# psaegert/bcnf

Hardware: AMD Instinct MI355X
Metric: NLL-training samples/sec + log_prob max-abs-err vs ref, trajectory_FC_small (higher is better)
Workload: dtype f32; 1 GPU; trajectory_FC_small NLL training step (configs[1]); batch_per_gpu=4096, global_batch=4096, parallelism=dp1, hip_graph=True, n_blocks=32, n_conditions=80

## Files before the change

bcnf_amd/csrc/bcnf_stack.hip:

```cpp
#include "bcnf_device.h"
#include "../../include/bcnf_amd.h"

#include <math.h>
#include <stdlib.h>
#include <string.h>

#include <algorithm>
#include <utility>
#include <vector>


#ifdef BCNF_PHASE_STAMPS
#define BCNF_STAMPS 1
#else
#define BCNF_STAMPS 0
#endif

namespace {

constexpr int NC16_MAX = 16;
constexpr int TILE = 256;
__host__ __device__ constexpr int tile_slot(int r, int q) { return 4 * r + ((q + (r >> 1)) & 3); }
__host__ __device__ constexpr int tile_ix(int s, int r) { return 4 * tile_slot(r, s & 3) + (s >> 2); }
__host__ __device__ constexpr int sample_of(int t8) { return (t8 >> 6) + 4 * ((t8 >> 4) & 3); }
// ... 855 lines not shown
#pragma unroll
    for (int e = 0; e < 8; ++e) {
      const int i4 = tid + 256 * e, r = i4 >> 5, col = (i4 & 31) * 4;
      if (col < L.Cp) *reinterpret_cast<floatx4*>(Bs + r * hs + col) = rv[e];
    }
#pragma unroll
    for (int kk = 0; kk < 2; ++kk) {
      const floatx4 v = va[kk] * am[kk];
#pragma unroll
      for (int q = 0; q < 4; ++q) As[(kk * 16 + j4 + q) * KHP + row] = v[q];
    }
    for (int c0 = KC; c0 < L.Cp; c0 += KC) {
      rows64_issue<VEC>(h, m1, L.C, L.ldh, m0 + KH * half, c0, rv);
      rows64_mask(m1, L.C, m0 + KH * half, c0, rv, ones);
#pragma unroll
      for (int e = 0; e < 8; ++e) {
        const int i4 = tid + 256 * e, r = i4 >> 5, col = c0 + (i4 & 31) * 4;
        if (col < L.Cp) *reinterpret_cast<floatx4*>(Bs + r * hs + col) = rv[e];
      }
    }
    __syncthreads();
#pragma unroll
    for (int j = 0; j < NT; ++j) {
      const int n = n_lo + j;
      if (n >= n_hi) continue;
#pragma unroll
      for (int t0 = 0; t0 < KH / 4; t0 += 8) {
        float a[8], bv[8];
#pragma unroll
        for (int t = 0; t < 8; ++t) {
          a[t] = As[(16 * kw + lr) * KHP + 4 * (t0 + t) + lq];
          bv[t] = Bs[(4 * (t0 + t) + lq) * hs + 16 * n + lr];
        }
#pragma unroll
        for (int t = 0; t < 8; t += 2) {
          acc[j] = mfma4(a[t], bv[t], acc[j]);
          acc1[j] = mfma4(a[t + 1], bv[t + 1], acc1[j]);
        }
      }
    }
  }
  if (k >= L.nb) return;
  float* o = work + (((long long)s * L.nb + k) * 16) * L.Cp;
#pragma unroll
  for (int j = 0; j < NT; ++j) {
    const int n = n_lo + j;
    if (n >= n_hi) continue;
    const floatx4 r = acc[j] + acc1[j];
#pragma unroll
    for (int i = 0; i < 4; ++i) o[(long long)(4 * lq + i) * L.Cp + 16 * n + lr] = r[i];
  }
}
size_t dw1h_half_lds_bytes(const BcnfLayout& L) {
  return sizeof(float) * (size_t)(32 * KHP + KH * bstride16(L.Cp));
}

__global__ __launch_bounds__(BCNF_WG) void k_dw1h_reduce(BcnfLayout L, const float* __restrict__ work, int splits,
                                                         float* __restrict__ dparams) {
  const long long per = 16LL * L.Cp, total = (long long)L.nb * per;
  const long long i = (long long)blockIdx.x * BCNF_WG + threadIdx.x;
  if (i >= total) return;
  const int k = (int)(i / per);
  const int rem = (int)(i - (long long)k * per);
  const int j = rem / L.Cp, c = rem - j * L.Cp;
  if (j >= L.H[1] || c >= L.C) return;
  float acc = 0.f;
  int s = 0;
  for (; s + 8 <= splits; s += 8) {
    float v[8];
#pragma unroll
    for (int t = 0; t < 8; ++t) v[t] = work[(long long)(s + t) * total + i];
#pragma unroll
    for (int t = 0; t < 8; ++t) acc += v[t];
  }
  for (; s < splits; ++s) acc += work[(long long)s * total + i];
  dparams[coupling_base(L, k) + L.lin_w[1] + j * L.lin_in[1] + L.Da + c] = acc;
}

__device__ __forceinline__ void gx_reduce_body(long long total, const float* __restrict__ work, int splits,
                                               float* __restrict__ gx, long long i) {
  if (i >= total) return;
  float acc = 0.f;
  int s = 0;
  for (; s + 16 <= splits; s += 16) {
    float v[16];
#pragma unroll
    for (int t = 0; t < 16; ++t) v[t] = work[(long long)(s + t) * total + i];
#pragma unroll
    for (int t = 0; t < 16; ++t) acc += v[t];
  }
  for (; s < splits; ++s) acc += work[(long long)s * total + i];
  gx[i] = acc;
}

__global__ __launch_bounds__(BCNF_WG) void k_fold_gx(long long total, const float* __restrict__ work, int splits,
                                                     float* __restrict__ gx) {
  gx_reduce_body(total, work, splits, gx, (long long)blockIdx.x * BCNF_WG + threadIdx.x);
}

struct RedShare {
  const float* slab;
  long long stride;
  int nwg;
  int own, first;
  float* dparams;
};
enum RedAdam { RED_NO_ADAM, RED_ADAM_DERIVED, RED_ADAM_PUBLISHED };
template <RedAdam AM>
__device__ __forceinline__ void reduce_share(const BcnfLayout& L, const RedShare& R, const FoldAdamArgs& A,
                                             float* __restrict__ smem);

__device__ __forceinline__ int c0_of_finish(int bx, int nct) { return (bx % nct) * 16; }

constexpr int FIN_KC = 512;
constexpr int FIN_SMEM = 2 * FIN_KC * 16;

__device__ __forceinline__ void tile16_accum(const float* __restrict__ As, const float* __restrict__ Bs, int kn,
                                             floatx4 (&acc)[4]) {
  const int lane = threadIdx.x & 63, ks = lane & 15, rb = lane >> 4, cb = threadIdx.x >> 6;
#pragma unroll 4
  for (int k = ks; k < kn; k += 16) {
    const floatx4 a = *reinterpret_cast<const floatx4*>(As + k * 16 + 4 * rb);
    const floatx4 b = *reinterpret_cast<const floatx4*>(Bs + k * 16 + 4 * cb);
#pragma unroll
    for (int r = 0; r < 4; ++r)
#pragma unroll
      for (int c = 0; c < 4; ++c) acc[r][c] = fmaf(a[r], b[c], acc[r][c]);
  }
}

__device__ __forceinline__ float tile16_reduce(float* __restrict__ red, const floatx4 (&acc)[4]) {
  const int lane = threadIdx.x & 63, ks = lane & 15, rb = lane >> 4, cb = threadIdx.x >> 6;
  __syncthreads();
#pragma unroll
  for (int r = 0; r < 4; ++r)
#pragma unroll
    for (int c = 0; c < 4; ++c) red[ks * 256 + (4 * rb + r) * 16 + 4 * cb + c] = acc[r][c];
  __syncthreads();
  float v = 0.f;
#pragma unroll
  for (int q = 0; q < 16; ++q) v += red[q * 256 + threadIdx.x];
  return v;
}

__global__ __launch_bounds__(BCNF_WG) void k_fold_finish(BcnfLayout L, const float* __restrict__ pk,
                                                         const float* __restrict__ gx, const float* __restrict__ wf,
                                                         const float* __restrict__ bf, int X,
                                                         float* __restrict__ dparams, float* __restrict__ dwf,
                                                         float* __restrict__ dbf, FoldAdamArgs A, RedShare R) {
  extern __shared__ __attribute__((aligned(16))) float smem[];
  if ((int)blockIdx.x >= R.own) {
    reduce_share<RED_ADAM_PUBLISHED>(L, R, A, smem);
    return;
  }
  float* As = smem;
  float* Bs = smem + FIN_KC * 16;
  const int Xp = fold_xp(X), tid = threadIdx.x, nct = L.Cp >> 4;
  floatx4 acc[4];
#pragma unroll
  for (int q = 0; q < 4; ++q) acc[q] = floatx4{0.f, 0.f, 0.f, 0.f};
  const bool adam = A.on && !(A.guard && A.guard[BCNF_GUARD_HALTED]);
  AdamScalars as{};
  const bool keeper = adam && blockIdx.x == 0 && tid == 0;
  const bool logger = keeper && A.log_values && A.log_history;
  long long log_row = 0;
  float step0 = 0.f, log_v[3];
  if (adam) {
    as = adam_scalars_of(A, A.asc[0], A.asc[1]);
    if (keeper) {
      log_row = A.cursor ? A.cursor[0] : 0LL;
      step0 = A.step[0];
    }
    if (logger) {
#pragma unroll
      for (int i = 0; i < 3; ++i) log_v[i] = A.log_values[i];
    }
  }
  int slot = -1;
  long long idx = 0;
  float ap = 0.f, am = 0.f, av = 0.f;
  if ((int)blockIdx.x < L.nb * nct) {
    const int j = tid >> 4, c = c0_of_finish(blockIdx.x, nct) + (tid & 15), k = blockIdx.x / nct;
    if (j < L.H[1] && c < L.C) {
      slot = 0;
      idx = coupling_base(L, k) + L.lin_w[1] + j * L.lin_in[1] + L.Da + c;
    }
  } else {
    const int tile = blockIdx.x - L.nb * nct, c = (tile % nct) * 16 + (tid >> 4), x = (tile / nct) * 16 + (tid & 15);
    if (c < L.C) {
      if (x < X) {
        slot = 1;
        idx = (long long)c * X + x;
      } else if (x == X && dbf) {
        slot = 2;
        idx = c;
      }
    }
  }
  float *sp = nullptr, *sm = nullptr, *sv = nullptr;
  if (adam) {
    if (slot == 0) {
      sp = A.p[0]; sm = A.m[0]; sv = A.v[0];
    } else if (slot == 1) {
      sp = A.p[1]; sm = A.m[1]; sv = A.v[1];
    } else if (slot == 2) {
      sp = A.p[2]; sm = A.m[2]; sv = A.v[2];
    }
  }
  if (sp) {
    ap = sp[idx];
    am = sm[idx];
    av = sv[idx];
  }
  auto finish_elem = [&](float gval) {
    if (!sp) return;
    adam_elem(ap, gval, am, av, as);
    sp[idx] = ap;
    sm[idx] = am;
    sv[idx] = av;
  };
  auto arrive = [&]() {
    if (!keeper) return;
    if (logger) __threadfence_system();
    A.step[0] = step0 + 1.0f;
    if (A.cursor) {
      const long long c = log_row + 1;
      A.cursor[0] = c < A.n_batches ? c : 0;
    }
  };
  if ((int)blockIdx.x < L.nb * nct) {
    const int k = blockIdx.x / nct, c0 = (blockIdx.x % nct) * 16;
    const float* g = gx + (long long)k * 16 * Xp;
    float va[16], vb[16];
#pragma unroll
    for (int e = 0; e < 16; ++e) {
      const int i = tid + BCNF_WG * e;
      const int j = i / Xp, xc = i - j * Xp, c = c0 + j;
      const bool in = i < 16 * Xp;
      va[e] = in ? g[i] : 0.f;
      float v = 0.f;
      if (in && c < L.C) v = xc < X ? wf[(long long)c * X + xc] : ((xc == X && bf) ? bf[c] : 0.f);
      vb[e] = v;
    }
#pragma unroll
    for (int e = 0; e < 16; ++e) {
      const int i = tid + BCNF_WG * e;
      if (i < 16 * Xp) {
        const int j = i / Xp, xc = i - j * Xp;
        As[xc * 16 + j] = va[e];
        Bs[xc * 16 + j] = vb[e];
      }
    }
    __syncthreads();
    if (logger) {
#pragma unroll
      for (int i = 0; i < 3; ++i)
        __hip_atomic_store(A.log_history + 3 * log_row + i, log_v[i], __ATOMIC_RELAXED, __HIP_MEMORY_SCOPE_SYSTEM);
    }
    tile16_accum(As, Bs, Xp, acc);
    const float v = tile16_reduce(smem, acc);
    const int j = tid >> 4, c = c0 + (tid & 15);
    if (j < L.H[1] && c < L.C) dparams[coupling_base(L, k) + L.lin_w[1] + j * L.lin_in[1] + L.Da + c] = v;
    finish_elem(v);
    __syncthreads();
    arrive();
    return;
  }
  const int tile = blockIdx.x - L.nb * nct, c0 = (tile % nct) * 16, x0 = (tile / nct) * 16;
  const int K = L.nb * 16;
  const float* w1r = pk + L.w1r_off + c0;
  for (int k0 = 0; k0 < K; k0 += FIN_KC) {
    const int kn = min(FIN_KC, K - k0);
    if (k0) __syncthreads();
    floatx4 va[FIN_KC * 4 / BCNF_WG], vb[FIN_KC * 4 / BCNF_WG];
#pragma unroll
    for (int e = 0; e < FIN_KC * 4 / BCNF_WG; ++e) {
      const int i4 = tid + BCNF_WG * e, r = i4 >> 2, q = i4 & 3, kj = k0 + (r < kn ? r : 0);
      va[e] = *reinterpret_cast<const floatx4*>(w1r + (long long)kj * L.Cp + 4 * q);
      vb[e] = *reinterpret_cast<const floatx4*>(gx + (long long)kj * Xp + x0 + 4 * q);
    }
#pragma unroll
    for (int e = 0; e < FIN_KC * 4 / BCNF_WG; ++e) {
      const int i4 = tid + BCNF_WG * e;
      reinterpret_cast<floatx4*>(As)[i4] = va[e];
      reinterpret_cast<floatx4*>(Bs)[i4] = vb[e];
    }
    __syncthreads();
    tile16_accum(As, Bs, kn, acc);
  }
  const float v = tile16_reduce(smem, acc);
  const int c = c0 + (tid >> 4), x = x0 + (tid & 15);
  if (c < L.C) {
    if (x < X) {
      if (dwf) dwf[(long long)c * X + x] = v;
    } else if (x == X && dbf) {
      dbf[c] = v;
    }
  }
  finish_elem(v);
  __syncthreads();
  arrive();
}

template <int NH>
struct RecF {
  static constexpr int B1 = 4, W1 = 8, HID = 24, T = 24 + 17 * (NH - 1), S = T + 17;
  static constexpr int Q = (S + 17 + 3) & ~3, MLP_END = (S + 17 + 3) & ~3, USED = Q + 64;
};
template <int NH>
struct RecB {
  static constexpr int AN = 0, QT = 4, TT = 68, ST = 84, HID = 100, W1T = 100 + 16 * (NH - 1);
  static constexpr int USED = W1T + 16;
};
template <int NH>
struct ActRec {
  static constexpr int YA = 2 * NH, YB = 2 * NH + 1, S = 2 * NH + 2;
  static constexpr int AR = 2 * NH + 3, AR4 = AR / 4, AR1 = AR - 4 * AR4;
  __host__ __device__ static constexpr int act(int l) { return 2 * l; }
  __host__ __device__ static constexpr int gd(int l) { return 2 * l + 1; }
  __host__ __device__ static constexpr int ready_layer(int q) {
    int r = 0;
    for (int i = 4 * q; i < 4 * q + 4; ++i) {
      const int li = i < 2 * NH ? i / 2 + 1 : (i == S ? NH + 1 : 0);
      r = li > r ? li : r;
    }
    return r;
  }
};

template <int LO, int HI>
__device__ __forceinline__ void ld_rec(float* __restrict__ rr, const float* __restrict__ R) {
  static_assert(LO % 4 == 0 && HI % 4 == 0, "record slices are 16-B aligned");
  const floatx4* R4 = reinterpret_cast<const floatx4*>(R + LO);
#pragma unroll
  for (int i = 0; i < (HI - LO) / 4; ++i) {
    const floatx4 v = R4[i];
    rr[LO + 4 * i + 0] = v.x;
// ... 1182 lines not shown
    for (int k = nb - 1; k >= 0; --k) {
      const int cur = k & 1;
      float gs[4 * BWD_G4];
      {
        const floatx4* gd4 = gsl + cur * BWD_G4 * BCNF_WG + tid;
#pragma unroll
        for (int i = 0; i < BWD_G4; ++i) {
          const floatx4 v = gd4[i * BCNF_WG];
          gs[4 * i] = v[0];
          gs[4 * i + 1] = v[1];
          gs[4 * i + 2] = v[2];
          gs[4 * i + 3] = v[3];
        }
      }
      float* Tt = dT + cur * J::ND * TILE + tix;
      const float* R = recB + cur * RING + j * L.RB;
      float rb[RBk::USED];
      ld_rec<0, RBk::HID>(rb, R);
      __builtin_amdgcn_sched_barrier(0);
      const float* gd = gs;
      const float S = gs[NH], ya = gs[NH + 1], yb = gs[NH + 2];
      const float an_sa = rb[RBk::AN], an_sb = rb[RBk::AN + 2], an_bb = rb[RBk::AN + 3];
      const float xb = fmaf(an_sb, yb, an_bb);
      const float e = exp_fast(S);
      float gza, gzb;
      if (QBC_DEV(L, QBC_MIX)) mix_bc(rb + RBk::QT, gya, gyb, gza, gzb);
      else mix(rb + RBk::QT, gya, gyb, gza, gzb);
      ld16(rb + RBk::HID, R + RBk::HID);
      __builtin_amdgcn_sched_barrier(0);
      const float dT_ = gzb;
      const float dS = (j < Db) ? fmaf(gzb * e, xb, dl) : 0.f;
      const float dSp = dS * (1.f - S * S);
      const float dxb = gzb * e;
      Tt[NH * TILE] = dT_;
      Tt[(NH + 1) * TILE] = dSp;
      float da = 0.f, da2 = 0.f;
      if (QBC_DEV(L, QBC_HEAD)) bc9x2(dT_, rb + RBk::TT, da, dSp, rb + RBk::ST, da2);
      else rot16x2(dT_, rb + RBk::TT, da, dSp, rb + RBk::ST, da2);
      da += da2;
#pragma unroll
      for (int l = NH; l >= 2; --l) {
        ld16(rb + RBk::HID + 16 * (NH - l + 1), R + RBk::HID + 16 * (NH - l + 1));
        __builtin_amdgcn_sched_barrier(0);
        const float dpre = da * gd[l - 1];
        Tt[(l - 1) * TILE] = dpre;
        da = rot16(dpre, rb + RBk::HID + 16 * (NH - l), 0.f);
      }
      const float dpre1 = da * gd[0];
      Tt[0] = dpre1;
      *(valid ? d1l + k * hps : d1_dummy) = dpre1;
      const float dxa = rot16(dpre1, rb + RBk::W1T, gza);
      {
        const float inv_a = (j < Da) ? __builtin_amdgcn_rcpf(an_sa) : 0.f;
        const float inv_b = (j < Db) ? __builtin_amdgcn_rcpf(an_sb) : 0.f;
        Tt[(NH + 2) * TILE] = fmaf(dxa, ya, dl * inv_a);
        Tt[(NH + 3) * TILE] = dxa;
        Tt[(NH + 4) * TILE] = fmaf(dxb, yb, dl * inv_b);
        Tt[(NH + 5) * TILE] = dxb;
      }
      gya = an_sa * dxa;
      gyb = an_sb * dxb;
      PHS(1)
      __syncthreads();
      PHS(2)
    }
    if (dy && valid) {
      if (j < Da) dy[b * D + j] = gya;
      if (j < Db) dy[b * D + Da + j] = gyb;
    }
  }
#if BCNF_STAMPS
  if (blockIdx.x == 0 && (threadIdx.x == 0 || threadIdx.x == BCNF_WG))
    for (int i = 0; i < 4; ++i) g_phase[(helper ? 4 : 0) + i] = ph_acc[i];
#endif
#undef PHS
  if (loss_out && blockIdx.x == 0) {
    __syncthreads();
    nll_finalize<BWD_WG>(nll_part, (int)gridDim.x, B, loss_out, rng_w, guard, dT);
  }
}

template <int N>
__device__ __forceinline__ int lpick(const int (&a)[N], int i) {
  int r = a[0];
#pragma unroll
  for (int t = 1; t < N; ++t) r = (i == t) ? a[t] : r;
  return r;
}

__device__ __forceinline__ long long slab_to_canonical(const BcnfLayout& L, int m, int o) {
  const int NH = L.NH, NW = NH + 2;
  const int cb = m * L.blk_stride + ((m < L.nb - 1) ? L.an_size : 0);
  if (o < NW * 256) {
    const int c = o >> 8, e = o & 255, lane = e >> 2;
    const int row = 4 * (lane >> 4) + (e & 3), col = lane & 15;
    const int l = c < NH ? c + 1 : NH + 1;
    const int nrows = c < NH ? lpick(L.H, l) : L.Db, ncols = (l == 1) ? L.Da : lpick(L.H, l - 1);
    if (row >= nrows || col >= ncols) return -1;
    const int row0 = (c == NH + 1) ? L.Db : 0;
    return (long long)cb + lpick(L.lin_w, l) + (row0 + row) * lpick(L.lin_in, l) + col;
  }
  const int o2 = o - NW * 256, c = o2 >> 4, r = o2 & 15;
  if (c < NH) return r < lpick(L.H, c + 1) ? (long long)cb + lpick(L.lin_b, c + 1) + r : -1;
  if (c < NH + 2) return r < L.Db ? (long long)cb + lpick(L.lin_b, NH + 1) + ((c == NH + 1) ? L.Db : 0) + r : -1;
  const int a = c - NH - 2;
  if (a >= 4 || !L.act_norm || m >= L.nb - 1 || r >= ((a < 2) ? L.Da : L.Db)) return -1;
  return (long long)m * L.blk_stride + ((a & 1) ? L.D : 0) + ((a < 2) ? 0 : L.Da) + r;
}

constexpr int RED_G = 8, RED_O4 = 32, RED_T = 16;

constexpr int RED_SMEM = RED_G * RED_O4 * 4 + 4;

template <RedAdam AM>
__device__ __forceinline__ void reduce_body(const BcnfLayout& L, const float* __restrict__ slab, long long stride,
                                            int nwg, float* __restrict__ out, int bx, float* __restrict__ smem,
                                            const FoldAdamArgs* A = nullptr) {
  floatx4 (*part)[RED_O4] = reinterpret_cast<floatx4 (*)[RED_O4]>(smem);
  float* sc = smem + RED_G * RED_O4 * 4;
  const int g = threadIdx.x / RED_O4, o4 = threadIdx.x % RED_O4;
  const long long i = ((long long)bx * RED_O4 + o4) * 4;
  const bool live = i < stride;
  const long long ic = live ? i : 0;
  const int m = (int)(ic / L.sblk), o = (int)(ic - (long long)m * L.sblk);
  long long ci[4];
  float ap[4], am[4], av[4];
  const float step0 = AM == RED_ADAM_DERIVED ? A->step[0] : 0.f;
  float pub[2] = {0.f, 0.f};
  if (AM == RED_ADAM_PUBLISHED && g == 0) {
    pub[0] = A->asc[0];
    pub[1] = A->asc[1];
  }
#pragma unroll
  for (int e = 0; e < 4; ++e) {
    ci[e] = slab_to_canonical(L, m, o + e);
    if (AM != RED_NO_ADAM && g == 0) {
      const long long c = ci[e] >= 0 ? ci[e] : 0;
      ap[e] = A->p[0][c];
      am[e] = A->m[0][c];
      av[e] = A->v[0][c];
    }
  }
  bool scalars_due = AM == RED_ADAM_DERIVED;
  auto scalars = [&]() {
    const double t = (double)(step0 + 1.0f);
    if (threadIdx.x == 0) sc[0] = (float)(A->lr / (1.0 - pow(A->b1, t)));
    if (threadIdx.x == 64) sc[1] = (float)sqrt(1.0 - pow(A->b2, t));
    scalars_due = false;
  };
  floatx4 acc = {0.f, 0.f, 0.f, 0.f};
  int w = g;
  for (; w + RED_G * (RED_T - 1) < nwg; w += RED_G * RED_T) {
    floatx4 v[RED_T];
#pragma unroll
    for (int t = 0; t < RED_T; ++t)
      v[t] = *reinterpret_cast<const floatx4*>(slab + (long long)(w + RED_G * t) * stride + ic);
    if (scalars_due) scalars();
#pragma unroll
    for (int t = 0; t < RED_T; ++t) acc += v[t];
  }
  for (; w < nwg; w += RED_G) acc += *reinterpret_cast<const floatx4*>(slab + (long long)w * stride + ic);
  if (scalars_due) scalars();
  part[g][o4] = acc;
  __syncthreads();
  if (g != 0 || !live) return;
  floatx4 tot = part[0][o4];
#pragma unroll
  for (int q = 1; q < RED_G; ++q) tot += part[q][o4];
  AdamScalars as{};
  if (AM == RED_ADAM_DERIVED) as = adam_scalars_of(*A, sc[0], sc[1]);
  if (AM == RED_ADAM_PUBLISHED) as = adam_scalars_of(*A, pub[0], pub[1]);
#pragma unroll
  for (int e = 0; e < 4; ++e) {
    if (ci[e] < 0) continue;
    out[ci[e]] = tot[e];
    if (AM != RED_NO_ADAM) {
      adam_elem(ap[e], tot[e], am[e], av[e], as);
      A->p[0][ci[e]] = ap[e];
      A->m[0][ci[e]] = am[e];
      A->v[0][ci[e]] = av[e];
    }
  }
}

template <RedAdam AM>
__device__ __forceinline__ void reduce_share(const BcnfLayout& L, const RedShare& R, const FoldAdamArgs& A,
                                             float* __restrict__ smem) {
  const int bx = R.first + ((int)blockIdx.x - R.own);
  if (A.on && !(A.guard && A.guard[BCNF_GUARD_HALTED])) {
    reduce_body<AM>(L, R.slab, R.stride, R.nwg, R.dparams, bx, smem, &A);
    return;
  }
  reduce_body<RED_NO_ADAM>(L, R.slab, R.stride, R.nwg, R.dparams, bx, smem);
}

struct TailGrid {
  int n_dh, gx_dh;
  int n_red;
  int gx_dw;
};

template <bool VEC>
__global__ __launch_bounds__(BCNF_WG) void k_bwd_tail(BcnfLayout L, TailGrid G, const float* __restrict__ pk,
                                                      const float* __restrict__ d1, const float* __restrict__ h,
                                                      long long B, float* __restrict__ dh,
                                                      const float* __restrict__ slab, long long stride, int nwg,
                                                      float* __restrict__ dparams, int rows_per_split,
                                                      float* __restrict__ work) {
  extern __shared__ __attribute__((aligned(16))) float smem[];
  int i = blockIdx.x;
  if (i < G.n_dh) {
    dh_body(L, pk, d1, B, dh, i % G.gx_dh, i / G.gx_dh, smem);
    return;
  }
  i -= G.n_dh;
  if (i < G.n_red) {
    reduce_body<RED_NO_ADAM>(L, slab, stride, nwg, dparams, i, smem);
    return;
  }
  i -= G.n_red;
  dw1h_body<VEC>(L, d1, h, B, rows_per_split, work, i % G.gx_dw, i / G.gx_dw, smem);
}

template <bool VEC, int NT>
__global__ __launch_bounds__(BCNF_WG, VEC && NT <= 3 ? 4 : 2) void k_fold_tail(BcnfLayout L, BcnfLayout F, const float* __restrict__ d1,
                                                       const float* __restrict__ x, long long B, int rows_per_split,
                                                       float* __restrict__ work, int gx_dw, int n_sk, int ones,
                                                       RedShare R, const float* __restrict__ wf,
                                                       const float* __restrict__ bf, float* __restrict__ wf1,
                                                       FoldAdamArgs A) {
  extern __shared__ __attribute__((aligned(16))) float smem[];
  const int bx = blockIdx.x;
  if (bx < n_sk) {
    dw1h_half_body<VEC, NT>(F, d1, x, B, rows_per_split, work, bx % gx_dw, bx / gx_dw, smem, ones);
    return;
  }
  if (bx == n_sk) {
    const int nw = L.C * F.C, n1 = nw + (bf ? L.C : 0);
    for (int i0 = 0; i0 < n1; i0 += 16 * BCNF_WG) {
      float v[16];
#pragma unroll
      for (int e = 0; e < 16; ++e) {
        const int i = min(i0 + e * BCNF_WG + (int)threadIdx.x, n1 - 1);
        v[e] = i < nw ? wf[i] : bf[i - nw];
      }
#pragma unroll
      for (int e = 0; e < 16; ++e) {
        const int i = i0 + e * BCNF_WG + (int)threadIdx.x;
        if (i < n1) wf1[i] = v[e];
      }
    }
    if (A.on && threadIdx.x == 0) adam_scalars_publish(A);
    return;
  }
  reduce_share<RED_ADAM_DERIVED>(L, R, A, smem);
}

__global__ __launch_bounds__(BCNF_WG) void k_fill_lds(float value) {
  extern __shared__ __attribute__((aligned(16))) float smem[];
  for (int i = threadIdx.x; i < (int)(LDS_MAX / 16); i += BCNF_WG)
    reinterpret_cast<floatx4*>(smem)[i] = floatx4{value, value, value, value};
  __syncthreads();
}

template <int NH>
bool layout_matches(const BcnfLayout& L) {
  return L.rf_b1 == RecF<NH>::B1 && L.rf_w1 == RecF<NH>::W1 && L.rf_hid == RecF<NH>::HID && L.rf_t == RecF<NH>::T &&
         L.rf_s == RecF<NH>::S && L.rf_q == RecF<NH>::Q && L.RF >= RecF<NH>::USED && L.rb_w1t == RecB<NH>::W1T &&
         L.rb_hid == RecB<NH>::HID && L.rb_tt == RecB<NH>::TT && L.rb_st == RecB<NH>::ST && L.rb_qt == RecB<NH>::QT &&
         L.rb_an == RecB<NH>::AN && L.RB >= RecB<NH>::USED;
}

bool vec_rows(const BcnfLayout& L, const float* h) { return L.ldh % 4 == 0 && ((uintptr_t)h & 15) == 0; }

int launch_hp(const BcnfLayout& L, const float* pk, const float* h, long long R, float* hp, hipStream_t st) {
  const size_t lds = hp_lds_bytes();
  const dim3 grid((unsigned)((R + 63) / 64), (unsigned)(L.NKp / 64));
  return vec_rows(L, h) ? launch<k_hp<true>>(grid, dim3(BCNF_WG), lds, st, L, pk, h, R, hp)
                        : launch<k_hp<false>>(grid, dim3(BCNF_WG), lds, st, L, pk, h, R, hp);
}

template <int NH>
int fwd_dispatch(const BcnfLayout& L, const float* pk, const float* y, const ProjArgs& P, long long B, float* z,
                 float* ldj, float* logp, bool drop, const uint64_t* rng, float* arec, float* part, hipStream_t st,
                 const RawArgs* raw = nullptr) {
  if (!layout_matches<NH>(L)) return BCNF_ERR_ARG;
  if (P.Cp % 16 != 0 || P.Cp / 16 > HP_SMAX || P.C > P.Cp) return BCNF_ERR_UNSUPPORTED;
  const dim3 grid((unsigned)((B + 15) / 16));
  const size_t lds = fwd2_lds_bytes(L, raw != nullptr);
  const bool save = arec != nullptr;
  const RawArgs R = raw ? *raw : RawArgs{};
#define FWD(DR, SV, RW) \
  launch<k_forward<NH, DR, SV, RW>>(grid, dim3(2 * BCNF_WG), lds, st, L, pk, y, P, B, z, ldj, logp, rng, arec, part, R)
  if (raw) return !save ? BCNF_ERR_ARG : drop ? FWD(true, true, true) : FWD(false, true, true);
  if (save) return drop ? FWD(true, true, false) : FWD(false, true, false);
  return drop ? FWD(true, false, false) : FWD(false, false, false);
#undef FWD
}

template <int NH>
int inv_dispatch(const BcnfLayout& L, const float* pk, const float* zin, const float* hp, long long R,
                 const int64_t* ci, long long N, float* y, bool drop, const uint64_t* rng, hipStream_t st) {
  if (!layout_matches<NH>(L)) return BCNF_ERR_ARG;
  if (!drop && L.RF == inv_m_rf<NH>() && L.PMB == (NH + 6) * 256 + (NH - 1) * 16 + 96) {
    const size_t lds_m = sizeof(float) * (size_t)(2 * RING);
    const dim3 grid_m((unsigned)((N + INV_M_SPB - 1) / INV_M_SPB));
    float* const none = nullptr;
    return L.Da <= 12 && L.Db <= 12
               ? launch<k_inverse_mfma<NH, true>>(grid_m, dim3(INV_M_WG), lds_m, st, L, pk, zin, hp, R, ci, N, y, none, none)
               : launch<k_inverse_mfma<NH, false>>(grid_m, dim3(INV_M_WG), lds_m, st, L, pk, zin, hp, R, ci, N, y, none, none);
  }
  const dim3 grid((unsigned)((N + 15) / 16));
  const size_t lds = fwd_lds_bytes(L);
  return drop ? launch<k_inverse<NH, true>>(grid, dim3(BCNF_WG), lds, st, L, pk, zin, hp, R, ci, N, y, rng)
              : launch<k_inverse<NH, false>>(grid, dim3(BCNF_WG), lds, st, L, pk, zin, hp, R, ci, N, y, rng);
}

template <int NH>
int inv_ldj_dispatch(const BcnfLayout& L, const float* pk, const float* zin, const float* hp, long long R,
                     const int64_t* ci, long long N, float* y, float* ldj, float* logp, hipStream_t st) {
  if (!layout_matches<NH>(L)) return BCNF_ERR_ARG;
  if (L.RF != inv_m_rf<NH>() || L.PMB != (NH + 6) * 256 + (NH - 1) * 16 + 96) return BCNF_ERR_UNSUPPORTED;
  const size_t lds_m = sizeof(float) * (size_t)(2 * RING);
  const dim3 grid_m((unsigned)((N + INV_M_SPB - 1) / INV_M_SPB));
  return L.Da <= 12 && L.Db <= 12
             ? launch<k_inverse_mfma<NH, true, true>>(grid_m, dim3(INV_M_WG), lds_m, st, L, pk, zin, hp, R, ci, N, y, ldj, logp)
             : launch<k_inverse_mfma<NH, false, true>>(grid_m, dim3(INV_M_WG), lds_m, st, L, pk, zin, hp, R, ci, N, y, ldj, logp);
}

long long slab_stride_of(const BcnfLayout& L) { return (long long)L.nb * L.sblk; }

template <int NH>
int bwd_dispatch(const BcnfLayout& L, const float* pk, const float* dz, const float* dldj, const float* dloss,
                 int nll, long long B, const float* arec, float* dy, float* d1, float* slab, long long stride,
                 const float* part, float* loss_out, uint64_t* rng_w, int32_t* guard, hipStream_t st) {
  if (!layout_matches<NH>(L)) return BCNF_ERR_ARG;
  const dim3 grid((unsigned)((B + 15) / 16));
  return launch<k_backward<NH>>(grid, dim3(BWD_WG), bwd_lds_bytes(L), st, L, pk, dz, dldj, dloss, nll, B, arec, dy, d1,
// ... 237 lines not shown
  const int npw = pack_wgs(L, true);
  const unsigned grid = (unsigned)(L.NKp / 16 * FOLD_SPLIT + ga.nwg + npw + 1);
  return launch<k_pack_fold>(dim3(grid), dim3(BCNF_WG), 0, (hipStream_t)stream, L, params, qmats, (float*)packed,
                             feat_weight, feat_bias, (int)in_features, fold, ga, npw);
}

int bcnf_fold_nll_forward(const BcnfStackDesc* desc, const void* packed, const float* fold, int32_t in_features,
                          const float* y, const float* x, int32_t ldx, int64_t batch, float* z, float* ldj, int32_t training,
                          uint64_t* rng_state, void* workspace, int32_t finalize, float* loss_out, int32_t* guard,
                          void* stream) {
  BcnfLayout L;
  const int rc = fold_setup(desc, in_features, &L);
  if (rc) return rc;
  if (!fold || ldx < in_features) return BCNF_ERR_ARG;
  return forward_impl(desc, packed, y, x, batch, z, ldj, nullptr, training, rng_state, workspace, true, true,
                      finalize != 0, loss_out, guard, stream, fold, in_features, ldx);
}

int bcnf_lds_fill(float value, void* stream) {
  return launch<k_fill_lds>(dim3(4 * 256), dim3(BCNF_WG), LDS_MAX, (hipStream_t)stream, value);
}

int bcnf_fold_raw_table_bytes(const BcnfStackDesc* desc, int32_t in_features, int64_t* bytes) {
  BcnfLayout L;
  const int rc = fold_setup(desc, in_features, &L);
  if (rc) return rc;
  if (!bytes) return BCNF_ERR_ARG;
  if (!raw_applicable(L, in_features)) return BCNF_ERR_UNSUPPORTED;
  std::vector<uint32_t> t((size_t)raw_table_words(L));
  if (!build_raw_table(L, t.data())) return BCNF_ERR_UNSUPPORTED;
  *bytes = (int64_t)t.size() * (int64_t)sizeof(uint32_t);
  return BCNF_OK;
}

int bcnf_fold_raw_table(const BcnfStackDesc* desc, int32_t in_features, void* host_table) {
  BcnfLayout L;
  const int rc = fold_setup(desc, in_features, &L);
  if (rc) return rc;
  if (!host_table) return BCNF_ERR_ARG;
  if (!raw_applicable(L, in_features)) return BCNF_ERR_UNSUPPORTED;
  return build_raw_table(L, (uint32_t*)host_table) ? BCNF_OK : BCNF_ERR_UNSUPPORTED;
}

int bcnf_fold_train_forward(const BcnfStackDesc* desc, const float* params, const float* qmats, const void* table,
                            const float* feat_weight, const float* feat_bias, int32_t in_features,
                            const BcnfGather2* gather, const float* y, const float* x, int32_t ldx, int64_t batch,
                            void* packed, float* z, float* ldj, int32_t training, uint64_t* rng_state,
                            void* workspace, int32_t finalize, float* loss_out, int32_t* guard, void* stream) {
  BcnfLayout L;
  const int rc = fold_setup(desc, in_features, &L);
  if (rc) return rc;
  if (!raw_applicable(L, in_features)) return BCNF_ERR_UNSUPPORTED;
  if (!params || !qmats || !table || !feat_weight || !packed || batch < 1) return BCNF_ERR_ARG;
  RawArgs R = {};
  R.P = params;
  R.Q = qmats;
  R.table = (const uint32_t*)table;
  R.wf = feat_weight;
  R.bf = feat_bias;
  R.pk = (float*)packed;
  R.X = in_features;
  if (gather) {
    const BcnfGather2& g = *gather;
    if (g.n != batch || g.cols0 != L.D || g.cols1 < in_features || !g.idx || !g.src0 || !g.src1 || !g.dst0 ||
        !g.dst1)
      return BCNF_ERR_ARG;
    R.idx = g.idx;
    R.cursor = (const long long*)g.cursor;
    R.ypool = g.src0;
    R.ydst = g.dst0;
    R.xpool = g.src1;
    R.xdst = g.dst1;
    R.ldx = g.cols1;
  } else {
    if (!y || !x || ldx < in_features) return BCNF_ERR_ARG;
    R.ypool = y;
    R.xpool = x;
    R.ldx = ldx;
  }
  return forward_impl(desc, packed, R.ypool, R.xpool, batch, z, ldj, nullptr, training, rng_state, workspace, true,
                      true, finalize != 0, loss_out, guard, stream, nullptr, 0, 0, &R);
}

constexpr int FOLD_RED_FIN_8THS = 2;
struct FoldTailPlan {
  long long S, splits;
  int n_red, gx_dw;
  int own[3];
  int first[3], count[3];
};
FoldTailPlan fold_tail_plan(const BcnfLayout& L, const BcnfLayout& F, int64_t batch) {
  FoldTailPlan P;
  P.S = slab_stride_of(L);
  P.splits = w1h_splits(batch);
  P.n_red = (int)((P.S / 4 + RED_O4 - 1) / RED_O4);
  P.gx_dw = (L.nb + 1) / 2;
  P.own[0] = (int)(P.gx_dw * P.splits) + 1;
  P.own[1] = (int)(((long long)L.nb * 16 * F.Cp + BCNF_WG - 1) / BCNF_WG);
  P.own[2] = (L.nb + (F.Cp >> 4)) * (L.Cp >> 4);
  P.count[1] = 0;
  P.count[2] = (int)((long long)P.n_red * FOLD_RED_FIN_8THS / 8);
  P.count[0] = P.n_red - P.count[2];
  P.first[0] = 0;
  P.first[1] = P.first[2] = P.count[0];
  return P;
}

int bcnf_fold_tail_plan(const BcnfStackDesc* desc, int32_t in_features, int64_t batch, int64_t* out) {
  BcnfLayout L;
  const int rc = fold_setup(desc, in_features, &L);
  if (rc) return rc;
  if (!out || batch < 1) return BCNF_ERR_ARG;
  const FoldTailPlan P = fold_tail_plan(L, fold_layout(L, in_features, in_features), batch);
  out[0] = P.n_red;
  out[1] = P.S;
  for (int t = 0; t < 3; ++t) {
    out[2 + 2 * t] = P.first[t];
    out[3 + 2 * t] = P.count[t];
    out[8 + t] = P.own[t] + P.count[t];
    out[11 + t] = P.own[t];
  }
  return BCNF_OK;
}

int bcnf_fold_backward_tail(const BcnfStackDesc* desc, const void* packed, const void* slab, const float* x,
                            int32_t ldx, int32_t in_features, const float* feat_weight, const float* feat_bias,
                            const void* workspace, int64_t batch, int32_t training, float* dparams,
                            float* dfeat_weight, float* dfeat_bias, const BcnfFoldAdam* adam, void* stream) {
  BcnfLayout L;
  int rc = fold_setup(desc, in_features, &L);
  if (rc) return rc;
  if (!packed || !slab || !x || !feat_weight || !workspace || !dparams || batch < 1 || ldx < in_features)
    return BCNF_ERR_ARG;
  FoldAdamArgs A = {};
  if (adam) {
    const BcnfFoldAdam& a = *adam;
    if (!a.params[0] || !a.exp_avg[0] || !a.exp_avg_sq[0] || !a.params[1] || !a.exp_avg[1] || !a.exp_avg_sq[1] ||
        !a.step || !a.done_counter || (feat_bias && (!a.params[2] || !a.exp_avg[2] || !a.exp_avg_sq[2])) ||
        (a.advance_cursor && a.cursor_modulo < 1))
      return BCNF_ERR_ARG;
    for (int t = 0; t < 3; ++t) {
      A.p[t] = a.params[t];
      A.m[t] = a.exp_avg[t];
      A.v[t] = a.exp_avg_sq[t];
    }
    if (!feat_bias) A.p[2] = A.m[2] = A.v[2] = nullptr;
    A.step = a.step;
    A.lr = a.lr;
    A.b1 = a.beta1;
    A.b2 = a.beta2;
    A.eps = a.eps;
    A.wd = a.weight_decay;
    A.cursor = (long long*)a.advance_cursor;
    A.n_batches = (long long)a.cursor_modulo;
    A.log_values = a.log_values;
    A.log_history = a.log_history;
    A.done = (int*)a.done_counter;
    A.guard = (const int*)a.guard;
    A.on = 1;
  }
  const BcnfLayout F = fold_layout(L, in_features, ldx);
  hipStream_t st = (hipStream_t)stream;
  const FoldTailPlan P = fold_tail_plan(L, F, batch);
  const long long S = P.S;
  const int nwg = (int)((batch + 15) / 16);
  const float* d1 = (const float*)workspace + ws_d1_off(L, batch);
  float* work = (float*)slab + (long long)nwg * S;
  float* gx = work + w1h_work_floats(F, batch);
  A.asc = gx + (long long)L.nb * 16 * F.Cp;
  const int rps = W1H_ROWS_PER_SPLIT;
  float* wf1 = A.asc + 4;
  const float* bf1 = feat_bias ? wf1 + (long long)L.C * in_features : nullptr;
  RedShare R[3];
  unsigned grid[3];
  for (int t = 0; t < 3; ++t) {
    R[t] = RedShare{(const float*)slab, S, nwg, P.own[t], P.first[t], dparams};
    grid[t] = (unsigned)(P.own[t] + P.count[t]);
  }
  const int n_sk = P.own[0] - 1;
  size_t lds = dw1h_half_lds_bytes(F);
  if (lds < sizeof(float) * RED_SMEM) lds = sizeof(float) * RED_SMEM;
  const bool vec = vec_rows(F, x);
  const bool nt3 = (F.Cp >> 4) <= 6;
#define FOLD_TAIL(V, NT)                                                                                          \
  launch<k_fold_tail<V, NT>>(dim3(grid[0]), dim3(BCNF_WG), lds, st, L, F, d1, x, (long long)batch, rps, work, P.gx_dw, \
                             n_sk, (int)in_features, R[0], feat_weight, feat_bias, wf1, A)
  rc = vec ? (nt3 ? FOLD_TAIL(true, 3) : FOLD_TAIL(true, 8)) : (nt3 ? FOLD_TAIL(false, 3) : FOLD_TAIL(false, 8));
#undef FOLD_TAIL
  if (rc) return rc;
  const long long total = (long long)L.nb * 16 * F.Cp;
  rc = launch<k_fold_gx>(dim3(grid[1]), dim3(BCNF_WG), 0, st, total, (const float*)work, (int)P.splits, gx);
  if (rc) return rc;
  return launch<k_fold_finish>(dim3(grid[2]), dim3(BCNF_WG), sizeof(float) * FIN_SMEM, st, L,
                               (const float*)packed, (const float*)gx, (const float*)wf1, bf1, (int)in_features,
                               dparams, dfeat_weight, dfeat_bias, A, R[2]);
}

int bcnf_grad_reduce(const BcnfStackDesc* desc, const void* slab, const float* h, const void* workspace,
                     int64_t batch, int32_t training, float* dparams, void* stream) {
  return bcnf_backward_tail(desc, slab, slab, h, workspace, batch, training, nullptr, dparams, stream);
}

int bcnf_stack_dh(const BcnfStackDesc* desc, const void* packed, const void* workspace, int64_t batch, int32_t training,
                  float* dh, void* stream) {
  BcnfLayout L;
  const int rc = stack_setup(desc, &L);
  if (rc) return rc;
  if (batch < 0 || !packed || !workspace || !dh) return BCNF_ERR_ARG;
  if (batch == 0) return BCNF_OK;
  const float* d1 = (const float*)workspace + ws_d1_off(L, batch);
  return launch<k_dh>(dim3((unsigned)((batch + 63) / 64), (unsigned)(L.Cp >> 4)), dim3(BCNF_WG), dh_lds_bytes(),
                      (hipStream_t)stream, L, (const float*)packed, d1, (long long)batch, dh);
}

int bcnf_stack_inverse(const BcnfStackDesc* desc, const void* packed, const float* z, const float* h, int64_t h_rows,
                       const int64_t* cond_index, int64_t n_rows, float* y, int32_t training,
                       const uint64_t* rng_state, void* scratch, void* stream) {
  BcnfLayout L;
  int rc = stack_setup(desc, &L);
  if (rc) return rc;
  if (n_rows == 0) return BCNF_OK;
  if (n_rows < 0 || h_rows < 1 || !packed || !z || !h || !y || !scratch) return BCNF_ERR_ARG;
  if (!cond_index && h_rows != n_rows) return BCNF_ERR_ARG;
  const bool drop = training && L.p > 0.f;
  if (drop && !rng_state) return BCNF_ERR_ARG;
  const float* pk = (const float*)packed;
  hipStream_t st = (hipStream_t)stream;
  float* hp = (float*)scratch;
  if ((rc = launch_hp(L, pk, h, h_rows, hp, st))) return rc;
  switch (L.NH) {
#define BCNF_CASE(N) case N: return inv_dispatch<N>(L, pk, z, hp, h_rows, cond_index, n_rows, y, drop, rng_state, st);
    BCNF_CASE(1) BCNF_CASE(2) BCNF_CASE(3) BCNF_CASE(4) BCNF_CASE(5) BCNF_CASE(6) BCNF_CASE(7) BCNF_CASE(8)
#undef BCNF_CASE
    default: return BCNF_ERR_UNSUPPORTED;
  }
}

int bcnf_stack_inverse_logdet(const BcnfStackDesc* desc, const void* packed, const float* z, const float* h,
                              int64_t h_rows, const int64_t* cond_index, int64_t n_rows, float* y, float* ldj,
                              float* log_prob, void* scratch, void* stream) {
  if (!desc) return BCNF_ERR_ARG;
  if (desc->two_way) return BCNF_ERR_UNSUPPORTED;
  if (!y || !ldj) return BCNF_ERR_ARG;
  BcnfLayout L;
  int rc = stack_setup(desc, &L);
  if (rc) return rc;
  if (n_rows == 0) return BCNF_OK;
  if (n_rows < 0 || h_rows < 1 || !packed || !z || !h || !scratch) return BCNF_ERR_ARG;
  if (!cond_index && h_rows != n_rows) return BCNF_ERR_ARG;
  const float* pk = (const float*)packed;
  hipStream_t st = (hipStream_t)stream;
  float* hp = (float*)scratch;
  if ((rc = launch_hp(L, pk, h, h_rows, hp, st))) return rc;
  switch (L.NH) {
#define BCNF_CASE(N) case N: return inv_ldj_dispatch<N>(L, pk, z, hp, h_rows, cond_index, n_rows, y, ldj, log_prob, st);
    BCNF_CASE(1) BCNF_CASE(2) BCNF_CASE(3) BCNF_CASE(4) BCNF_CASE(5) BCNF_CASE(6) BCNF_CASE(7) BCNF_CASE(8)
#undef BCNF_CASE
    default: return BCNF_ERR_UNSUPPORTED;
  }
}

const char* bcnf_status_string(int status) {
  switch (status) {
    case BCNF_OK: return "ok";
    case BCNF_ERR_ARG: return "invalid argument";
    case BCNF_ERR_UNSUPPORTED: return "unsupported stack shape for the fused kernel family";
    default: return status >= BCNF_ERR_HIP_BASE ? hipGetErrorString((hipError_t)(status - BCNF_ERR_HIP_BASE))
                                                 : "unknown status";
  }
}

#if BCNF_STAMPS
int bcnf_debug_phases(unsigned long long* out) {
  return bcnf_rt::hip_status(hipMemcpyFromSymbol(out, HIP_SYMBOL(g_phase), sizeof(g_phase)));
// ... 43 lines not shown
```

Measured before the change: 31.89 million samples/s.

## Let gx fold kernel take a reduction share and deepen reduction load batches

Gives k_fold_gx the ability to run a share of the slab reduction with Adam, like k_fold_finish, and adds a configurable share plan (set to zero by default). Reduction loops in k_fold_finish and k_fold_gx now issue 32 loads per round before accumulating, and the gx reduce body also gets a 32-wide unrolled path. The halted-guard check moves from a skip of Adam to a per-element gate using relaxed atomic loads, and lpick becomes an OR-select. Deeper batches raise register pressure in exchange for more memory-level parallelism.

New measurement: 32.14 million samples/s, median of 6. About the same (+0.8%).

```diff
diff --git a/bcnf_amd/csrc/bcnf_stack.hip b/bcnf_amd/csrc/bcnf_stack.hip
--- a/bcnf_amd/csrc/bcnf_stack.hip
+++ b/bcnf_amd/csrc/bcnf_stack.hip
@@ -961,6 +961,13 @@
   if (i >= total) return;
   float acc = 0.f;
   int s = 0;
+  for (; s + 32 <= splits; s += 32) {
+    float v[32];
+#pragma unroll
+    for (int t = 0; t < 32; ++t) v[t] = work[(long long)(s + t) * total + i];
+#pragma unroll
+    for (int t = 0; t < 32; ++t) acc += v[t];
+  }
   for (; s + 16 <= splits; s += 16) {
     float v[16];
 #pragma unroll
@@ -970,11 +977,6 @@
   }
   for (; s < splits; ++s) acc += work[(long long)s * total + i];
   gx[i] = acc;
-}
-
-__global__ __launch_bounds__(BCNF_WG) void k_fold_gx(long long total, const float* __restrict__ work, int splits,
-                                                     float* __restrict__ gx) {
-  gx_reduce_body(total, work, splits, gx, (long long)blockIdx.x * BCNF_WG + threadIdx.x);
 }
 
 struct RedShare {
@@ -985,9 +987,28 @@
   float* dparams;
 };
 enum RedAdam { RED_NO_ADAM, RED_ADAM_DERIVED, RED_ADAM_PUBLISHED };
-template <RedAdam AM>
+
+template <typename T>
+__device__ __forceinline__ T load_word_v(const T* p) {
+  return __hip_atomic_load(p, __ATOMIC_RELAXED, __HIP_MEMORY_SCOPE_AGENT);
+}
+__device__ __forceinline__ int guard_halted(const int* guard) {
+  return guard ? load_word_v(guard + BCNF_GUARD_HALTED) : 0;
+}
+
+template <RedAdam AM, int RT>
 __device__ __forceinline__ void reduce_share(const BcnfLayout& L, const RedShare& R, const FoldAdamArgs& A,
                                              float* __restrict__ smem);
+
+__global__ __launch_bounds__(BCNF_WG) void k_fold_gx(BcnfLayout L, long long total, const float* __restrict__ work,
+                                                     int splits, float* __restrict__ gx, FoldAdamArgs A, RedShare R) {
+  extern __shared__ __attribute__((aligned(16))) float smem[];
+  if ((int)blockIdx.x >= R.own) {
+    reduce_share<RED_ADAM_PUBLISHED, 32>(L, R, A, smem);
+    return;
+  }
+  gx_reduce_body(total, work, splits, gx, (long long)blockIdx.x * BCNF_WG + threadIdx.x);
+}
 
 __device__ __forceinline__ int c0_of_finish(int bx, int nct) { return (bx % nct) * 16; }
 
@@ -1029,7 +1050,7 @@
                                                          float* __restrict__ dbf, FoldAdamArgs A, RedShare R) {
   extern __shared__ __attribute__((aligned(16))) float smem[];
   if ((int)blockIdx.x >= R.own) {
-    reduce_share<RED_ADAM_PUBLISHED>(L, R, A, smem);
+    reduce_share<RED_ADAM_PUBLISHED, 32>(L, R, A, smem);
     return;
   }
   float* As = smem;
@@ -1038,14 +1059,15 @@
   floatx4 acc[4];
 #pragma unroll
   for (int q = 0; q < 4; ++q) acc[q] = floatx4{0.f, 0.f, 0.f, 0.f};
-  const bool adam = A.on && !(A.guard && A.guard[BCNF_GUARD_HALTED]);
+  const bool adam = A.on;
+  const int halted = adam ? guard_halted(A.guard) : 0;
   AdamScalars as{};
   const bool keeper = adam && blockIdx.x == 0 && tid == 0;
   const bool logger = keeper && A.log_values && A.log_history;
   long long log_row = 0;
   float step0 = 0.f, log_v[3];
   if (adam) {
-    as = adam_scalars_of(A, A.asc[0], A.asc[1]);
+    as = adam_scalars_of(A, load_word_v(A.asc), load_word_v(A.asc + 1));
     if (keeper) {
       log_row = A.cursor ? A.cursor[0] : 0LL;
       step0 = A.step[0];
@@ -1092,14 +1114,14 @@
     av = sv[idx];
   }
   auto finish_elem = [&](float gval) {
-    if (!sp) return;
+    if (!sp || halted) return;
     adam_elem(ap, gval, am, av, as);
     sp[idx] = ap;
     sm[idx] = am;
     sv[idx] = av;
   };
   auto arrive = [&]() {
-    if (!keeper) return;
+    if (!keeper || halted) return;
     if (logger) __threadfence_system();
     A.step[0] = step0 + 1.0f;
     if (A.cursor) {
@@ -1131,7 +1153,7 @@
       }
     }
     __syncthreads();
-    if (logger) {
+    if (logger && !halted) {
 #pragma unroll
       for (int i = 0; i < 3; ++i)
         __hip_atomic_store(A.log_history + 3 * log_row + i, log_v[i], __ATOMIC_RELAXED, __HIP_MEMORY_SCOPE_SYSTEM);
@@ -2480,9 +2502,9 @@
 
 template <int N>
 __device__ __forceinline__ int lpick(const int (&a)[N], int i) {
-  int r = a[0];
-#pragma unroll
-  for (int t = 1; t < N; ++t) r = (i == t) ? a[t] : r;
+  int r = 0;
+#pragma unroll
+  for (int t = 0; t < N; ++t) r |= (i == t) ? a[t] : 0;
   return r;
 }
 
@@ -2508,9 +2530,20 @@
 
 constexpr int RED_G = 8, RED_O4 = 32, RED_T = 16;
 
+template <int T>
+__device__ __forceinline__ void red_issue(floatx4 (&v)[T], const float* __restrict__ base, long long stride) {
+#pragma unroll
+  for (int t = 0; t < T; ++t) v[t] = *reinterpret_cast<const floatx4*>(base + (long long)(RED_G * t) * stride);
+}
+template <int T>
+__device__ __forceinline__ void red_add(floatx4& acc, const floatx4 (&v)[T]) {
+#pragma unroll
+  for (int t = 0; t < T; ++t) acc += v[t];
+}
+
 constexpr int RED_SMEM = RED_G * RED_O4 * 4 + 4;
 
-template <RedAdam AM>
+template <RedAdam AM, int RT = RED_T>
 __device__ __forceinline__ void reduce_body(const BcnfLayout& L, const float* __restrict__ slab, long long stride,
                                             int nwg, float* __restrict__ out, int bx, float* __restrict__ smem,
                                             const FoldAdamArgs* A = nullptr) {
@@ -2523,15 +2556,18 @@
   const int m = (int)(ic / L.sblk), o = (int)(ic - (long long)m * L.sblk);
   long long ci[4];
   float ap[4], am[4], av[4];
-  const float step0 = AM == RED_ADAM_DERIVED ? A->step[0] : 0.f;
+  static_assert(RT == RED_T || RT == 2 * RED_T, "rounds of RT, then of RED_T, then single slabs");
+  const float step0 = AM == RED_ADAM_DERIVED ? load_word_v(A->step) : 0.f;
+  const int halted = AM != RED_NO_ADAM ? guard_halted(A->guard) : 0;
   float pub[2] = {0.f, 0.f};
   if (AM == RED_ADAM_PUBLISHED && g == 0) {
-    pub[0] = A->asc[0];
-    pub[1] = A->asc[1];
-  }
+    pub[0] = load_word_v(A->asc);
+    pub[1] = load_word_v(A->asc + 1);
+  }
+#pragma unroll
+  for (int e = 0; e < 4; ++e) ci[e] = slab_to_canonical(L, m, o + e);
 #pragma unroll
   for (int e = 0; e < 4; ++e) {
-    ci[e] = slab_to_canonical(L, m, o + e);
     if (AM != RED_NO_ADAM && g == 0) {
       const long long c = ci[e] >= 0 ? ci[e] : 0;
       ap[e] = A->p[0][c];
@@ -2548,14 +2584,19 @@
   };
   floatx4 acc = {0.f, 0.f, 0.f, 0.f};
   int w = g;
-  for (; w + RED_G * (RED_T - 1) < nwg; w += RED_G * RED_T) {
-    floatx4 v[RED_T];
-#pragma unroll
-    for (int t = 0; t < RED_T; ++t)
-      v[t] = *reinterpret_cast<const floatx4*>(slab + (long long)(w + RED_G * t) * stride + ic);
+  for (; w + RED_G * (RT - 1) < nwg; w += RED_G * RT) {
+    floatx4 v[RT];
+    red_issue(v, slab + (long long)w * stride + ic, stride);
     if (scalars_due) scalars();
-#pragma unroll
-    for (int t = 0; t < RED_T; ++t) acc += v[t];
+    red_add(acc, v);
+  }
+  if (RT > RED_T) {
+    for (; w + RED_G * (RED_T - 1) < nwg; w += RED_G * RED_T) {
+      floatx4 v[RED_T];
+      red_issue(v, slab + (long long)w * stride + ic, stride);
+      if (scalars_due) scalars();
+      red_add(acc, v);
+    }
   }
   for (; w < nwg; w += RED_G) acc += *reinterpret_cast<const floatx4*>(slab + (long long)w * stride + ic);
   if (scalars_due) scalars();
@@ -2572,7 +2613,7 @@
   for (int e = 0; e < 4; ++e) {
     if (ci[e] < 0) continue;
     out[ci[e]] = tot[e];
-    if (AM != RED_NO_ADAM) {
+    if (AM != RED_NO_ADAM && !halted) {
       adam_elem(ap[e], tot[e], am[e], av[e], as);
       A->p[0][ci[e]] = ap[e];
       A->m[0][ci[e]] = am[e];
@@ -2581,15 +2622,15 @@
   }
 }
 
-template <RedAdam AM>
+template <RedAdam AM, int RT>
 __device__ __forceinline__ void reduce_share(const BcnfLayout& L, const RedShare& R, const FoldAdamArgs& A,
                                              float* __restrict__ smem) {
   const int bx = R.first + ((int)blockIdx.x - R.own);
-  if (A.on && !(A.guard && A.guard[BCNF_GUARD_HALTED])) {
-    reduce_body<AM>(L, R.slab, R.stride, R.nwg, R.dparams, bx, smem, &A);
+  if (A.on) {
+    reduce_body<AM, RT>(L, R.slab, R.stride, R.nwg, R.dparams, bx, smem, &A);
     return;
   }
-  reduce_body<RED_NO_ADAM>(L, R.slab, R.stride, R.nwg, R.dparams, bx, smem);
+  reduce_body<RED_NO_ADAM, RT>(L, R.slab, R.stride, R.nwg, R.dparams, bx, smem);
 }
 
 struct TailGrid {
@@ -2651,7 +2692,7 @@
     if (A.on && threadIdx.x == 0) adam_scalars_publish(A);
     return;
   }
-  reduce_share<RED_ADAM_DERIVED>(L, R, A, smem);
+  reduce_share<RED_ADAM_DERIVED, RED_T>(L, R, A, smem);
 }
 
 __global__ __launch_bounds__(BCNF_WG) void k_fill_lds(float value) {
@@ -3055,7 +3096,7 @@
                       true, finalize != 0, loss_out, guard, stream, nullptr, 0, 0, &R);
 }
 
-constexpr int FOLD_RED_FIN_8THS = 2;
+constexpr int FOLD_RED_GX_8THS = 0, FOLD_RED_FIN_8THS = 2;
 struct FoldTailPlan {
   long long S, splits;
   int n_red, gx_dw;
@@ -3071,11 +3112,14 @@
   P.own[0] = (int)(P.gx_dw * P.splits) + 1;
   P.own[1] = (int)(((long long)L.nb * 16 * F.Cp + BCNF_WG - 1) / BCNF_WG);
   P.own[2] = (L.nb + (F.Cp >> 4)) * (L.Cp >> 4);
-  P.count[1] = 0;
+  static_assert(FOLD_RED_GX_8THS >= 0 && FOLD_RED_FIN_8THS >= 0 && FOLD_RED_GX_8THS + FOLD_RED_FIN_8THS < 8,
+                "k_fold_tail keeps a share");
+  P.count[1] = (int)((long long)P.n_red * FOLD_RED_GX_8THS / 8);
   P.count[2] = (int)((long long)P.n_red * FOLD_RED_FIN_8THS / 8);
-  P.count[0] = P.n_red - P.count[2];
+  P.count[0] = P.n_red - P.count[1] - P.count[2];
   P.first[0] = 0;
-  P.first[1] = P.first[2] = P.count[0];
+  P.first[1] = P.count[0];
+  P.first[2] = P.count[0] + P.count[1];
   return P;
 }
 
@@ -3162,7 +3206,8 @@
 #undef FOLD_TAIL
   if (rc) return rc;
   const long long total = (long long)L.nb * 16 * F.Cp;
-  rc = launch<k_fold_gx>(dim3(grid[1]), dim3(BCNF_WG), 0, st, total, (const float*)work, (int)P.splits, gx);
+  rc = launch<k_fold_gx>(dim3(grid[1]), dim3(BCNF_WG), sizeof(float) * RED_SMEM, st, L, total, (const float*)work,
+                         (int)P.splits, gx, A, R[1]);
   if (rc) return rc;
   return launch<k_fold_finish>(dim3(grid[2]), dim3(BCNF_WG), sizeof(float) * FIN_SMEM, st, L,
                                (const float*)packed, (const float*)gx, (const float*)wf1, bf1, (int)in_features,
```
